# CDACHPCIE25/PPQSFLHE

Measured on AMD Instinct MI355X. Metric: ciphertexts/sec aggregated+PRE at N=2^16, L=12 RNS limbs, higher is better.
Workload: dtype u64

## Files before the change

include/mkckks.h:

```cpp
#ifndef MKCKKS_H
#define MKCKKS_H

#include <stddef.h>
#include <stdint.h>

#ifdef __cplusplus
extern "C" {
#endif

#define MKCKKS_OK 0
#define MKCKKS_E_INVALID (-1)
#define MKCKKS_E_NODEVICE (-2)
#define MKCKKS_E_HIP (-3)
#define MKCKKS_E_NOMEM (-4)
#define MKCKKS_E_INTERNAL (-5)
#define MKCKKS_E_PRECISION (-6)

typedef struct mkckks_ctx mkckks_ctx;

typedef struct mkckks_params {
    uint32_t log_n;
    uint32_t mult_depth;
    uint32_t scaling_bits;
    uint32_t first_bits;
// ... 32 lines not shown
int mkckks_host_free(mkckks_ctx *c, void *h_ptr);
int mkckks_upload_async(mkckks_ctx *c, void *d_dst, const void *h_src_pinned, size_t bytes, uint64_t *ticket_out);
int mkckks_download_async(mkckks_ctx *c, void *h_dst_pinned, const void *d_src, size_t bytes, uint64_t *ticket_out);
int mkckks_copy_done(mkckks_ctx *c, uint64_t ticket, int *done_out);
int mkckks_copy_wait(mkckks_ctx *c, uint64_t ticket);
int mkckks_fence_uploads(mkckks_ctx *c);
int mkckks_fence_compute(mkckks_ctx *c);
int mkckks_count_noncanonical(mkckks_ctx *c, const uint64_t *d_ct, uint32_t n_ct, uint32_t nl, uint64_t *h_count);

int mkckks_ntt_forward_batch(mkckks_ctx *c, uint64_t *d_polys, uint32_t n_polys, uint32_t nl, int with_p);
int mkckks_ntt_inverse_batch(mkckks_ctx *c, uint64_t *d_polys, uint32_t n_polys, uint32_t nl, int with_p);

int mkckks_eval_add_batch(mkckks_ctx *c, const uint64_t *d_a, const uint64_t *d_b, uint64_t *d_out,
                          uint32_t n_ct, uint32_t nl);
int mkckks_eval_sum_batch(mkckks_ctx *c, const uint64_t *d_in, uint64_t *d_out, uint32_t n_clients,
                          uint32_t n_ct, uint32_t nl);

int mkckks_rescale_mult_const_batch(mkckks_ctx *c, const uint64_t *d_in, uint64_t *d_out, uint32_t n_ct,
                                    uint32_t nl, double operand);
int mkckks_rescale_batch(mkckks_ctx *c, const uint64_t *d_in, uint64_t *d_out, uint32_t n_ct, uint32_t nl);
int mkckks_mult_const_batch(mkckks_ctx *c, uint64_t *d_ct, uint32_t n_ct, uint32_t nl, double operand);

int mkckks_mult_plain_batch(mkckks_ctx *c, uint64_t *d_ct, const uint64_t *d_pt, uint32_t n_ct, uint32_t n_pt, uint32_t nl);
int mkckks_mult_plain_rescale_batch(mkckks_ctx *c, const uint64_t *d_in, const uint64_t *d_pt, uint64_t *d_out, uint32_t n_ct,
                                    uint32_t n_pt, uint32_t nl);

int mkckks_reencrypt_batch(mkckks_ctx *c, const uint64_t *d_ct, const uint64_t *d_evk, uint64_t *d_out,
                           uint32_t n_ct, uint32_t nl);
int mkckks_reencrypt_accumulate_batch(mkckks_ctx *c, const uint64_t *d_ct, const uint64_t *d_evk, uint64_t *d_acc,
                                      uint32_t n_ct, uint32_t nl);
int mkckks_reencrypt_sum_batch(mkckks_ctx *c, const uint64_t *d_cts, const uint64_t *d_evks, uint64_t *d_out,
                               uint32_t n_clients, uint32_t n_ct, uint32_t nl);
int mkckks_q0_walk_choice(uint32_t row_tiles, uint32_t n_int_q, uint32_t n_idx, int mode);
int mkckks_scale_evk_batch(mkckks_ctx *c, const uint64_t *d_evk_in, uint64_t *d_evk_out, uint32_t n_keys,
                           const double *h_weights, uint32_t sf_level);
int mkckks_reencrypt_wsum_batch(mkckks_ctx *c, const uint64_t *d_cts, const uint64_t *d_evks_scaled, uint64_t *d_out,
                                uint32_t n_clients, uint32_t n_ct, uint32_t nl, const double *h_weights, uint32_t sf_level);
int mkckks_eval_wsum_batch(mkckks_ctx *c, const uint64_t *d_in, uint64_t *d_out, uint32_t n_terms, uint32_t n_ct, uint32_t nl,
                           const double *h_weights, uint32_t sf_level, int first_is_sum);
int mkckks_reencrypt_fanout_batch(mkckks_ctx *c, const uint64_t *d_ct, const uint64_t *d_evks, uint64_t *d_out,
                                  uint32_t n_keys, uint32_t n_ct, uint32_t nl);
int mkckks_compress_batch(mkckks_ctx *c, const uint64_t *d_in, uint64_t *d_out, uint32_t n_ct, uint32_t nl_in,
                          uint32_t nl_out);
int mkckks_reencrypt_fanout_compact_batch(mkckks_ctx *c, const uint64_t *d_ct, const uint64_t *d_evks, uint64_t *d_out,
                                          uint32_t n_keys, uint32_t n_ct, uint32_t nl_in, uint32_t nl_out);
int mkckks_modup_batch(mkckks_ctx *c, const uint64_t *d_c1, uint64_t *d_digits, uint32_t n, uint32_t nl);
int mkckks_moddown_batch(mkckks_ctx *c, const uint64_t *d_in, uint64_t *d_out, uint32_t n, uint32_t nl);

#define MKCKKS_SAMPLER_KEY_BYTES 32
int mkckks_sample_ternary(mkckks_ctx *c, int8_t *d_out, size_t count, const uint8_t *h_key32, uint32_t stream_id);
int mkckks_sample_gauss(mkckks_ctx *c, int32_t *d_out, size_t count, double sigma, const uint8_t *h_key32,
                        uint32_t stream_id);
int mkckks_sample_uniform(mkckks_ctx *c, uint64_t *d_out, uint32_t n_polys, uint32_t nl, int with_p,
                          const uint8_t *h_key32, uint32_t stream_id);
int mkckks_sample_gauss_wide(mkckks_ctx *c, int64_t *d_out, size_t count, double sigma, const uint8_t *h_key32,
                             uint32_t stream_id);
int mkckks_chacha20_block(mkckks_ctx *c, uint32_t *d_out16, const uint8_t *h_key32, uint32_t counter,
                          const uint32_t *h_nonce3);

int mkckks_keygen(mkckks_ctx *c, const int8_t *d_s, const uint64_t *d_a, const int32_t *d_e,
                  uint64_t *d_pk, uint64_t *d_sk);
int mkckks_rekeygen(mkckks_ctx *c, const int8_t *d_s_old, const uint64_t *d_pk_new, const int8_t *d_u,
                    const int32_t *d_e0, const int32_t *d_e1, uint64_t *d_evk);

int mkckks_encrypt_batch(mkckks_ctx *c, const uint64_t *d_pk, const uint64_t *d_pt, const int8_t *d_v,
                         const int32_t *d_e0, const int32_t *d_e1, uint64_t *d_ct, uint32_t n_ct, uint32_t nl);
// ... 100 lines not shown
```

ppqsflhe_amd/binding.py:

```python
import ctypes as C
import os

import numpy as np

_HERE = os.path.dirname(os.path.abspath(__file__))
_LIB = os.environ.get("MKCKKS_LIB") or os.path.join(_HERE, "libmkckks_hip.so")


class MkckksError(RuntimeError):
    def __init__(self, code, msg):
        super().__init__(f"mkckks error {code}: {msg}")
        self.code = code


class _Params(C.Structure):
    _fields_ = [("log_n", C.c_uint32), ("mult_depth", C.c_uint32), ("scaling_bits", C.c_uint32),
                ("first_bits", C.c_uint32), ("dnum", C.c_uint32), ("aux_bits", C.c_uint32),
                ("extra_bits", C.c_uint32), ("device", C.c_int32)]


class _Info(C.Structure):
    _fields_ = [("ring_dim", C.c_uint32), ("num_q", C.c_uint32), ("num_p", C.c_uint32),
                ("alpha", C.c_uint32), ("beta", C.c_uint32), ("slots", C.c_uint32)]

# ... 25 lines not shown
    "mkckks_fence_compute": (_int, [_vp]),
    "mkckks_count_noncanonical": (_int, [_vp, _vp, _u32, _u32, C.POINTER(C.c_uint64)]),
    "mkckks_debug_stamps": (_int, [_vp, _vp, _u32, C.POINTER(_sz)]),
    "mkckks_ntt_forward_batch": (_int, [_vp, _vp, _u32, _u32, _int]),
    "mkckks_ntt_inverse_batch": (_int, [_vp, _vp, _u32, _u32, _int]),
    "mkckks_eval_add_batch": (_int, [_vp, _vp, _vp, _vp, _u32, _u32]),
    "mkckks_eval_sum_batch": (_int, [_vp, _vp, _vp, _u32, _u32, _u32]),
    "mkckks_rescale_mult_const_batch": (_int, [_vp, _vp, _vp, _u32, _u32, _dbl]),
    "mkckks_rescale_batch": (_int, [_vp, _vp, _vp, _u32, _u32]),
    "mkckks_mult_const_batch": (_int, [_vp, _vp, _u32, _u32, _dbl]),
    "mkckks_mult_plain_batch": (_int, [_vp, _vp, _vp, _u32, _u32, _u32]),
    "mkckks_mult_plain_rescale_batch": (_int, [_vp, _vp, _vp, _vp, _u32, _u32, _u32]),
    "mkckks_reencrypt_batch": (_int, [_vp, _vp, _vp, _vp, _u32, _u32]),
    "mkckks_reencrypt_accumulate_batch": (_int, [_vp, _vp, _vp, _vp, _u32, _u32]),
    "mkckks_reencrypt_sum_batch": (_int, [_vp, _vp, _vp, _vp, _u32, _u32, _u32]),
    "mkckks_reencrypt_fanout_batch": (_int, [_vp, _vp, _vp, _vp, _u32, _u32, _u32]),
    "mkckks_scale_evk_batch": (_int, [_vp, _vp, _vp, _u32, _vp, _u32]),
    "mkckks_reencrypt_wsum_batch": (_int, [_vp, _vp, _vp, _vp, _u32, _u32, _u32, _vp, _u32]),
    "mkckks_eval_wsum_batch": (_int, [_vp, _vp, _vp, _u32, _u32, _u32, _vp, _u32, _int]),
    "mkckks_compress_batch": (_int, [_vp, _vp, _vp, _u32, _u32, _u32]),
    "mkckks_reencrypt_fanout_compact_batch": (_int, [_vp, _vp, _vp, _vp, _u32, _u32, _u32, _u32]),
    "mkckks_modup_batch": (_int, [_vp, _vp, _vp, _u32, _u32]),
    "mkckks_moddown_batch": (_int, [_vp, _vp, _vp, _u32, _u32]),
    "mkckks_keygen": (_int, [_vp, _vp, _vp, _vp, _vp, _vp]),
    "mkckks_rekeygen": (_int, [_vp, _vp, _vp, _vp, _vp, _vp, _vp]),
    "mkckks_keygen_join": (_int, [_vp, _vp, _vp, _vp, _vp, _vp]),
    "mkckks_partial_decrypt_batch": (_int, [_vp, _vp, _vp, _vp, _vp, _u32, _u32, _u32, _int]),
    "mkckks_fuse_shares_batch": (_int, [_vp, _vp, _vp, _u32, _u32, _u32]),
    "mkckks_switch_share_batch": (_int, [_vp, _vp, _vp, _vp, _vp, _vp, _vp, _vp, _u32, _u32, _u32, _int]),
    "mkckks_share_key": (_int, [_vp, _vp, _vp, _u32, _u32, _u32, C.c_char_p, _u32]),
    "mkckks_combine_key_shares": (_int, [_vp, _vp, _vp, _vp, _u32, _u32]),
    "mkckks_lagrange_at_zero": (_int, [_vp, _vp, _u32, _vp]),
    "mkckks_q0_walk_choice": (_int, [_u32, _u32, _u32, _int]),
    "mkckks_encrypt_batch": (_int, [_vp, _vp, _vp, _vp, _vp, _vp, _vp, _u32, _u32]),
    "mkckks_lift_ntt_batch": (_int, [_vp, _vp, _vp, _u32, _u32]),
    "mkckks_decrypt_batch": (_int, [_vp, _vp, _vp, _vp, _u32, _u32]),
    "mkckks_sample_ternary": (_int, [_vp, _vp, _sz, C.c_char_p, _u32]),
    "mkckks_sample_gauss": (_int, [_vp, _vp, _sz, _dbl, C.c_char_p, _u32]),
    "mkckks_sample_gauss_wide": (_int, [_vp, _vp, _sz, _dbl, C.c_char_p, _u32]),
    "mkckks_rerandomize_batch": (_int, [_vp, _vp, _vp, _vp, _vp, _vp, _vp, _u32, _u32, _u32]),
    "mkckks_sample_uniform": (_int, [_vp, _vp, _u32, _u32, _int, C.c_char_p, _u32]),
    "mkckks_chacha20_block": (_int, [_vp, _vp, C.c_char_p, _u32, C.POINTER(_u32)]),
    "mkckks_encrypt_seeded_batch": (_int, [_vp, _vp, _vp, _vp, _vp, _u32, _u32, C.c_char_p, _u32]),
    "mkckks_expand_seeded_batch": (_int, [_vp, _vp, _u32, _u32, C.c_char_p, C.POINTER(_u32)]),
    "mkckks_encode_batch": (_int, [_vp, _vp, _vp, _u32, _u32, _dbl]),
    "mkckks_decode_batch": (_int, [_vp, _vp, _vp, _u32, _u32, _dbl]),
    "mkckks_decode_flood_batch": (_int, [_vp, _vp, _vp, _u32, _u32, _dbl, C.c_char_p, _u32, _vp]),
    "mkckks_reduce_mod_batch": (_int, [_vp, _vp, _u32, _u32, _u32]),
    "mkckks_comm_unique_id": (_int, [_vp]),
    "mkckks_comm_create": (_int, [_vp, _vp, _int, _int, C.POINTER(_vp)]),
    "mkckks_comm_destroy": (_int, [_vp, _vp]),
    "mkckks_reduce_scatter_sum_mod": (_int, [_vp, _vp, _vp, _vp, _u32, _u32, _u32]),
    "mkckks_comm_library": (C.c_char_p, []),
    "mkckks_ctx_twiddles": (_int, [_vp, _u32, _int, _u64p]),
    "mkckks_debug_arith": (_int, [_vp, _u32, C.c_uint64, _vp, _vp, _sz]),
}
ARITH_OPS = {
    "csub": (0, 2, 1, 0),
    "add_mod": (1, 2, 1, 0),
    "sub_mod": (2, 2, 1, 0),
    "shoup_lazy": (3, 2, 1, 1),
    "shoup_mul": (4, 2, 1, 1),
    "mul_mod": (5, 2, 1, 0),
    "barrett_reduce128": (6, 2, 1, 0),
    "reduce_wide": (7, 2, 1, 0),
    "reduce_word": (8, 1, 1, 0),
# ... 474 lines not shown
```

ppqsflhe_amd/csrc/capi.cpp:

```cpp
#include <cstring>
#include <new>
#include <string>

#include "../../include/mkckks.h"
#include "comm.hpp"
#include "engine.hpp"

struct mkckks_ctx {
    mk::Engine *eng;
};

namespace {
thread_local std::string g_err;

template <typename F>
int guarded(F &&f) {
    try {
        f();
        return MKCKKS_OK;
    } catch (const mk::PrecisionError &e) {
        g_err = e.what();
        return MKCKKS_E_PRECISION;
    } catch (const mk::NoDevice &e) {
        g_err = e.what();
// ... 275 lines not shown
                                    uint32_t n_pt, uint32_t nl) {
    return guarded([&] {
        need(c && in && pt && out, "null argument");
        need(nl >= 2 && nl <= c->eng->params().L, "nl out of range");
        need(n_pt == 1 || n_pt == n_ct, "n_pt must be 1 or n_ct");
        c->eng->mult_plain_rescale(in, pt, out, n_ct, n_pt, nl);
    });
}

int mkckks_reencrypt_batch(mkckks_ctx *c, const uint64_t *ct, const uint64_t *evk, uint64_t *out, uint32_t n_ct,
                           uint32_t nl) {
    return guarded([&] {
        need(c && ct && evk && out, "null argument");
        c->eng->reencrypt(ct, evk, out, n_ct, nl);
    });
}
int mkckks_reencrypt_accumulate_batch(mkckks_ctx *c, const uint64_t *ct, const uint64_t *evk, uint64_t *acc,
                                      uint32_t n_ct, uint32_t nl) {
    return guarded([&] {
        need(c && ct && evk && acc, "null argument");
        c->eng->reencrypt(ct, evk, acc, n_ct, nl, true);
    });
}
int mkckks_reencrypt_sum_batch(mkckks_ctx *c, const uint64_t *cts, const uint64_t *evks, uint64_t *out, uint32_t n_clients,
                               uint32_t n_ct, uint32_t nl) {
    return guarded([&] {
        need(c && cts && evks && out, "null argument");
        c->eng->reencrypt_sum(cts, evks, out, n_clients, n_ct, nl);
    });
}
int mkckks_q0_walk_choice(uint32_t row_tiles, uint32_t n_int_q, uint32_t n_idx, int mode) {
    return mk::q0_walk_fused(row_tiles, n_int_q, n_idx, mode) ? 1 : 0;
}
int mkckks_scale_evk_batch(mkckks_ctx *c, const uint64_t *d_evk_in, uint64_t *d_evk_out, uint32_t n_keys,
                           const double *h_weights, uint32_t sf_level) {
    return guarded([&] {
        need(c && (n_keys == 0 || (d_evk_in && d_evk_out && h_weights)), "null argument");
        c->eng->scale_evk(d_evk_in, d_evk_out, n_keys, h_weights, sf_level);
    });
}
int mkckks_reencrypt_wsum_batch(mkckks_ctx *c, const uint64_t *d_cts, const uint64_t *d_evks_scaled, uint64_t *d_out,
                                uint32_t n_clients, uint32_t n_ct, uint32_t nl, const double *h_weights, uint32_t sf_level) {
    return guarded([&] {
        need(c && ((n_clients == 0 || n_ct == 0) || (d_cts && d_evks_scaled && d_out && h_weights)), "null argument");
        c->eng->reencrypt_wsum(d_cts, d_evks_scaled, d_out, n_clients, n_ct, nl, h_weights, sf_level);
    });
}
int mkckks_eval_wsum_batch(mkckks_ctx *c, const uint64_t *d_in, uint64_t *d_out, uint32_t n_terms, uint32_t n_ct, uint32_t nl,
                           const double *h_weights, uint32_t sf_level, int first_is_sum) {
    return guarded([&] {
        need(c && ((n_terms == 0 || n_ct == 0) || (d_in && d_out && h_weights)), "null argument");
        c->eng->eval_wsum(d_in, d_out, n_terms, n_ct, nl, h_weights, sf_level, first_is_sum != 0);
    });
}
int mkckks_reencrypt_fanout_batch(mkckks_ctx *c, const uint64_t *ct, const uint64_t *evks, uint64_t *out, uint32_t n_keys,
                                  uint32_t n_ct, uint32_t nl) {
    return guarded([&] {
        need(c && ct && evks && out, "null argument");
        need(nl >= 1 && nl <= c->eng->params().L, "nl out of range");
        if (!n_keys || !n_ct) return;
        c->eng->reencrypt_fanout(ct, evks, out, n_keys, n_ct, nl);
    });
}
static void need_compact_args(const mk::ParamSet &ps, const uint64_t *in, const uint64_t *out, uint32_t n_keys, uint32_t n_ct,
                              uint32_t nl_in, uint32_t nl_out) {
    need(nl_out >= 1 && nl_out < nl_in && nl_in <= ps.L, "need 1 <= nl_out < nl_in <= L");
// ... 292 lines not shown
```

ppqsflhe_amd/csrc/engine.hip:

```cpp
#include "engine.hpp"
#include "comm.hpp"
#include "dispatch.hpp"
#include "ntt_radix.hpp"
#include "qsum_kernels.hpp"
#include "fanout_kernels.hpp"
#include "codec_kernels.hpp"
#include "sampler_kernels.hpp"
#include "arith_probe_kernels.hpp"
#include "../../include/mkckks.h"

#include <cmath>
#include <cstdio>
#include <type_traits>
#include <cstdlib>
#include <cstring>

namespace mk {


template <bool INV>
__global__ __launch_bounds__(NTT_THREADS) void k_ntt_col(NttIo io, NttTables T, const u64 *scale,
                                                         const u64 *scale_sh) {
    extern __shared__ __attribute__((aligned(16))) u64 lds[];
    const uint32_t poly = blockIdx.y / io.nslots, s = blockIdx.y % io.nslots;
    if (ntt_slot_skipped(io, poly, io.vslot0 + s)) return;
    const uint32_t id = limb_id_of(io.vslot0 + s, io.nl, T.L);
    const LimbConst lc = T.limb[id];
    const uint32_t n = 1u << T.log_n, r1 = 1u << T.log_r1, r2 = 1u << T.log_r2;
    const u64 *src = io.in + (size_t)poly * io.in_stride + (size_t)(io.in_slot0 + s) * n;
    u64 *dst = io.out + (size_t)poly * io.out_stride + (size_t)(io.out_slot0 + s) * n;
    const uint32_t c0 = blockIdx.x * NTT_COLS;
    const uint32_t pairs = r1 * (NTT_COLS / 2);
    for (uint32_t e = threadIdx.x; e < pairs; e += NTT_THREADS) {
        const uint32_t r = e / (NTT_COLS / 2), cp = (e % (NTT_COLS / 2)) * 2;
        const ulong2 v = *reinterpret_cast<const ulong2 *>(src + (size_t)r * r2 + c0 + cp);
        lds[r * NTT_COLS + cp] = v.x;
        lds[r * NTT_COLS + cp + 1] = v.y;
    }
    __syncthreads();
    const u64 *tw = (INV ? T.itw : T.tw) + (size_t)id * n;
    const u64 *tw_sh = (INV ? T.itw_sh : T.tw_sh) + (size_t)id * n;
    lds_stages<INV>(lds, NTT_COLS, (int)T.log_r1, 1, NTT_COLS, true, tw, tw_sh, lc.q, lc.q2,
                    [](int) { return 1; });
// ... 466 lines not shown
    return msg + "): the one initialised second sees no device -- load the library that owns the device first (import torch "
                 "before libmkckks_hip.so, or link both against the same libamdhip64)";
}

static bool env_flag(const char *name, bool dflt) {
    const char *e = std::getenv(name);
    return e ? std::atoi(e) != 0 : dflt;
}
Knobs Knobs::from_env() {
    Knobs k;
    if (const char *e = std::getenv("MKCKKS_CHUNK")) {
        const int v = std::atoi(e);
        if (v >= 1 && v <= 64) k.chunk = (uint32_t)v;
    }
    if (const char *e = std::getenv("MKCKKS_QSUM_GROUP")) {
        const int v = std::atoi(e);
        if (v >= 1 && v <= 64) k.qsum_group = (uint32_t)v;
    }
    if (const char *e = std::getenv("MKCKKS_FANOUT_GROUP")) {
        const int v = std::atoi(e);
        if (v >= 1 && v <= 64) k.fanout_group = (uint32_t)v;
    }
    k.cu_affine = env_flag("MKCKKS_CU_AFFINE", k.cu_affine);
    k.generic_ntt = env_flag("MKCKKS_GENERIC_NTT", k.generic_ntt);
    k.no_pm = env_flag("MKCKKS_NO_PM", k.no_pm);
    k.no_fp64 = env_flag("MKCKKS_NO_FP64", k.no_fp64);
    if (const char *e = std::getenv("MKCKKS_Q0_WALK")) {
        if (!std::strcmp(e, "0")) k.q0_walk = 0;
        else if (!std::strcmp(e, "1")) k.q0_walk = 1;
    }
    if (const char *e = std::getenv("MKCKKS_PLAIN_FUSED")) {
        if (!std::strcmp(e, "0")) k.plain_fused = 0;
        else if (!std::strcmp(e, "1")) k.plain_fused = 1;
    }
    return k;
}

Engine::Engine(const ParamSet &ps, int device) : ps_(ps), device_(device), knobs_(Knobs::from_env()) {
    if (device_ < 0) return;
    int count = 0;
    if (hipGetDeviceCount(&count) != hipSuccess || count <= device_)
        throw NoDevice("no HIP device " + std::to_string(device_) + " (found " + std::to_string(count) + ")" +
                       hip_runtime_diagnosis());
    MK_HIP(hipSetDevice(device_));
    const uint32_t D = ps_.D, n = ps_.n;
    tabs_.log_n = ps_.log_n;
    tabs_.log_r1 = (ps_.log_n % 2 == 0) ? ((ps_.log_n / 2) & ~1u) : ps_.log_n / 2;
    tabs_.log_r2 = ps_.log_n - tabs_.log_r1;
    if (knobs_.generic_ntt) { tabs_.log_r1 = ps_.log_n / 2; tabs_.log_r2 = ps_.log_n - tabs_.log_r1; }
    const bool radix_both = fast_log_h(tabs_.log_r1, 1u << tabs_.log_r2) && fast_row(tabs_.log_r2, 1u << tabs_.log_r1);
    const bool fp_ok = radix_both && !knobs_.no_fp64;
    tabs_.has_fp = 0;
    fp_of_.assign(D, 0);
    for (uint32_t i = 0; i < D; ++i) {
        ps_.limb[i].fp = (fp_ok && ps_.moduli[i] < (5ull << 48)) ? 1u : 0u;
        fp_of_[i] = (uint8_t)ps_.limb[i].fp;
        tabs_.has_fp |= ps_.limb[i].fp;
    }
    bool all_pm = radix_both && !knobs_.no_pm;
    for (uint32_t i = 0; i < D; ++i)
        if (!ps_.limb[i].fp && !pm_eligible(ps_.moduli[i])) all_pm = false;
    tabs_.int_pm = all_pm ? 1u : 0u;
    for (uint32_t i = 0; i < D; ++i) {
        const bool pm = all_pm && !ps_.limb[i].fp;
        ps_.limb[i].pm = pm ? 1u : 0u;
        ps_.limb[i].pm_c = pm ? (uint32_t)(((u64)1 << ps_.limb[i].k) - ps_.moduli[i]) : 0u;
// ... 338 lines not shown
    ClassMasks m;
    if (classes & 1) m.integer = class_mask(io, T.h_fp_of, T.L, false);
    if (classes & 2) m.fp = class_mask(io, T.h_fp_of, T.L, true);
    return m;
}
static ClassMasks limb_classes(uint32_t nl, const NttTables &T) {
    NttIo sel{};
    sel.nslots = sel.nl = nl;
    return slot_classes(sel, T);
}
static ClassMasks target_classes(const DevConv &cv, const NttTables &T, unsigned classes = 3) {
    ClassMasks m;
    for (uint32_t j = 0; j < cv.n_out; ++j) {
        const bool fp = T.h_fp_of[cv.dst_id[j]] != 0;
        if (fp && (classes & 2)) m.fp |= 1ull << j;
        if (!fp && (classes & 1)) m.integer |= 1ull << j;
    }
    return m;
}

template <typename F>
static void for_each_class(const NttTables &T, const ClassMasks &m, F &&f) {
    if (m.integer) with_int_arith(T, [&](auto ar) { f(ar, m.integer, (uint32_t)__builtin_popcountll(m.integer)); });
    if (m.fp) f(std::integral_constant<int, AR_FP>{}, m.fp, (uint32_t)__builtin_popcountll(m.fp));
}

template <int LOG_H>
static uint32_t col_tiles(const NttTables &T) { return (1u << T.log_r2) / (256u >> LOG_H); }
template <int LOG_H>
static uint32_t row_tiles(const NttTables &T) { return (1u << T.log_r1) / (256u >> LOG_H); }

template <bool INV>
static void launch_col(const NttIo &io0, const NttTables &T, uint32_t n_polys, const u64 *scale, const u64 *scale_sh,
                       hipStream_t s, int pack = 0) {
    const uint32_t r1 = 1u << T.log_r1, r2 = 1u << T.log_r2;
    const bool radix = dispatch<2, 3, 4>(fast_log_h(T.log_r1, r2), [&](auto log_h) {
        constexpr int LOG_H = decltype(log_h)::value;
        for_each_class(T, slot_classes(io0, T), [&](auto ar, unsigned long long mask, uint32_t nsel) {
            NttIo io = io0;
            io.slot_mask = mask;
            io.nsel = nsel;
            k_ntt_col_r<LOG_H, INV, decltype(ar)::value>
                <<<dim3(col_tiles<LOG_H>(T), n_polys * nsel), NTT_THREADS, 0, s>>>(io, T, scale, scale_sh, pack);
        });
    });
    if (radix) return;
    if (pack) throw std::logic_error("packed output needs the radix column kernel");
    k_ntt_col<INV><<<dim3(r2 / NTT_COLS, n_polys * io0.nslots), NTT_THREADS, (size_t)r1 * NTT_COLS * sizeof(u64), s>>>(
        io0, T, scale, scale_sh);
}

static bool row_tail_supported(const NttTables &T) { return fast_row(T.log_r2, 1u << T.log_r1) != 0; }

template <bool INV>
static void launch_row(const NttIo &io0, const NttTables &T, uint32_t n_polys, const TailArgs &tail, hipStream_t s,
                       unsigned classes = 3) {
    const uint32_t n = 1u << T.log_n, r1 = 1u << T.log_r1;
    const bool radix = dispatch<2, 3, 4, 9>(fast_row(T.log_r2, r1), [&](auto row_h) {
        constexpr int ROW_H = decltype(row_h)::value;
        for_each_class(T, slot_classes(io0, T, classes), [&](auto ar, unsigned long long mask, uint32_t nsel) {
            NttIo io = io0;
            io.slot_mask = mask;
            io.nsel = nsel;
            if constexpr (ROW_H == 9)
                k_ntt_row3<INV, decltype(ar)::value><<<dim3((r1 / 4) * n_polys * nsel), NTT_THREADS, 0, s>>>(io, T, tail);
            else
                k_ntt_row_r<ROW_H, INV, decltype(ar)::value>
                    <<<dim3(row_tiles<ROW_H>(T) * n_polys * nsel), NTT_THREADS, 0, s>>>(io, T, tail);
        });
    });
    if (radix) return;
    if (tail.enabled) throw std::logic_error("fused tail needs the radix row kernel");
    const uint32_t tile = n < (uint32_t)NTT_TILE ? n : (uint32_t)NTT_TILE;
    k_ntt_row<INV><<<dim3(n / tile, n_polys * io0.nslots), NTT_THREADS, (size_t)tile * sizeof(u64), s>>>(io0, T);
}

static void ntt_passes(NttIo io, const NttTables &T, uint32_t n_polys, bool inverse, const u64 *scale,
                       const u64 *scale_sh, hipStream_t s, int pack = 0) {
    if (n_polys == 0 || io.nslots == 0) return;
    NttIo second = io;
    second.in_group = 0;
    second.in = io.out;
    second.in_stride = io.out_stride;
    second.in_slot0 = io.out_slot0;
    const TailArgs none{};
    if (!inverse) {
        launch_col<false>(io, T, n_polys, nullptr, nullptr, s);
        launch_row<false>(second, T, n_polys, none, s);
    } else {
        launch_row<true>(io, T, n_polys, none, s);
        launch_col<true>(second, T, n_polys, scale, scale_sh, s, pack);
    }
    MK_HIP(hipGetLastError());
}

template <int LOG_H, int N_IN, int SRCMODE>
static void launch_conv_col_n(const ConvIo &io0, const NttTables &T, const DevConv &cv, hipStream_t s, unsigned classes) {
    for_each_class(T, target_classes(cv, T, classes), [&](auto ar, unsigned long long mask, uint32_t nsel) {
        ConvIo io = io0;
        io.target_mask = mask;
        io.nsel = nsel;
        if constexpr (LOG_H >= 3)
            k_conv_col2<LOG_H, N_IN, decltype(ar)::value, DevConv, SRCMODE>
                <<<dim3(io.items * col_tiles<LOG_H>(T) * ((nsel + 1) / 2)), NTT_THREADS, 0, s>>>(io, T, cv);
        else
            k_conv_col<LOG_H, N_IN, decltype(ar)::value, DevConv, SRCMODE>
                <<<dim3(io.items * col_tiles<LOG_H>(T) * nsel), NTT_THREADS, 0, s>>>(io, T, cv);
    });
}
template <int LOG_H, int N_IN>
static void launch_conv_col_m(const ConvIo &io, const NttTables &T, const DevConv &cv, hipStream_t s, int srcmode,
                              unsigned classes) {
    if constexpr (N_IN <= 4 && LOG_H >= 3) {
        if (srcmode == 1) return launch_conv_col_n<LOG_H, N_IN, 1>(io, T, cv, s, classes);
        if (srcmode == 2) return launch_conv_col_n<LOG_H, N_IN, (N_IN > 1 ? 2 : 0)>(io, T, cv, s, classes);
    }
    if (srcmode != 0) throw std::logic_error("double conversion sources: unsupported shape");
    launch_conv_col_n<LOG_H, N_IN, 0>(io, T, cv, s, classes);
}
static bool launch_conv_col(const ConvIo &io, const NttTables &T, const DevConv &cv, hipStream_t s, int srcmode = 0,
                            unsigned classes = 3) {
    const bool radix = dispatch<2, 3, 4>(fast_log_h(T.log_r1, 1u << T.log_r2), [&](auto log_h) {
        if (!dispatch<1, 2, 3, 4, 5, 6, 7, 8>(cv.n_in, [&](auto n_in) {
                launch_conv_col_m<decltype(log_h)::value, decltype(n_in)::value>(io, T, cv, s, srcmode, classes);
            }))
            throw std::invalid_argument("base conversion fan-in unsupported");
    });
    if (radix) MK_HIP(hipGetLastError());
    return radix;
}
template <int LOG_H, int N_IN>
static void launch_conv_col_psum_n(const ConvIo &io0, const NttTables &T, const DevConv &cv, hipStream_t s) {
    for_each_class(T, target_classes(cv, T), [&](auto ar, unsigned long long mask, uint32_t nsel) {
        ConvIo io = io0;
        io.target_mask = mask;
        io.nsel = nsel;
        if constexpr (decltype(ar)::value == AR_FP)
            k_conv_col_psum2<LOG_H, N_IN, DevConv>
                <<<dim3(io.items * col_tiles<LOG_H>(T) * ((nsel + 1) / 2)), NTT_THREADS, 0, s>>>(io, T, cv);
        else
            k_conv_col_psum<LOG_H, N_IN, decltype(ar)::value, DevConv>
                <<<dim3(io.items * col_tiles<LOG_H>(T) * nsel), NTT_THREADS, 0, s>>>(io, T, cv);
    });
}
static void launch_conv_col_psum(const ConvIo &io, const NttTables &T, const DevConv &cv, hipStream_t s) {
    if (!dispatch<3, 4>(fast_log_h(T.log_r1, 1u << T.log_r2), [&](auto log_h) {
            if (!dispatch<1, 2, 3, 4, 5, 6, 7, 8>(cv.n_in, [&](auto n_in) {
                    launch_conv_col_psum_n<decltype(log_h)::value, decltype(n_in)::value>(io, T, cv, s);
                }))
                throw std::invalid_argument("base conversion fan-in unsupported");
        }))
        throw std::logic_error("summed conversion needs 64- or 256-point columns");
    MK_HIP(hipGetLastError());
}
static void launch_icol_sum(const u64 *pc, u64 *psum, const NttTables &T, uint32_t K, uint32_t n_polys, uint32_t n_clients,
                            size_t in_cstride, hipStream_t s) {
    if (!dispatch<3, 4>(fast_log_h(T.log_r1, 1u << T.log_r2), [&](auto log_h) {
            constexpr int LOG_H = decltype(log_h)::value;
            with_int_arith(T, [&](auto ar) {
                k_icol_sum<LOG_H, decltype(ar)::value><<<dim3(col_tiles<LOG_H>(T), n_polys * K), NTT_THREADS, 0, s>>>(
                    pc, psum, T, K, n_clients, in_cstride);
            });
// ... 273 lines not shown
        for (size_t i = 0; i < t.src.size(); ++i) put(t.src[i], t.hatinv[i]);
    }
    BaseConvTable t = ps_.moddown_table(nl);
    for (size_t i = 0; i < t.src.size(); ++i) put(t.src[i], t.hatinv[i]);
    return limb_vector(key, v);
}

const u64 *Engine::p_inverse(uint32_t nl) {
    const std::string key = "pinv_" + std::to_string(nl);
    auto it = vec_cache_.find(key);
    if (it != vec_cache_.end()) return it->second;
    std::vector<u64> pinv(2 * nl);
    for (uint32_t i = 0; i < nl; ++i) {
        pinv[i] = ps_.p_inv_mod(i);
        pinv[nl + i] = h_shoup(pinv[i], ps_.moduli[i]);
    }
    return limb_vector(key, pinv);
}

void Engine::modup_core(const u64 *c1, size_t c1_stride, u64 *coef, u64 *dig, uint32_t cnt, uint32_t nl,
                        bool rows_int_only, uint32_t in_group, size_t in_gstride, bool p_scaled) {
    const uint32_t n = ps_.n, ext = nl + ps_.K, nparts = ps_.num_parts(nl), D = ps_.D;
    const u64 *fold = folded_scale(nl);
    bool fused = fast_log_h(tabs_.log_r1, 1u << tabs_.log_r2) != 0;
    NttIo s1{c1, coef, c1_stride, (size_t)nl * n, 0, 0, 0, nl, nl};
    s1.in_group = in_group;
    s1.in_gstride = in_gstride;
    const size_t dstride = (size_t)nparts * ext * n;
    bool doubles = fused && tabs_.has_fp && fast_log_h(tabs_.log_r1, 1u << tabs_.log_r2) >= 3;
    for (uint32_t part = 0; part < nparts && doubles; ++part) {
        const DevConv &cv = modup_conv(nl, part, p_scaled);
        if (conv_src_mode(cv) < 0 || (conv_src_mode(cv) != 0 && cv.n_in > 4)) doubles = false;
    }
    ntt_passes(s1, tabs_, cnt, true, fold, fold + D, stream_, fused ? (doubles ? 2 : 1) : 0);
    for (uint32_t part = 0; part < nparts && fused; ++part) {
        ConvIo io{coef, dig + (size_t)part * ext * n, (size_t)nl * n, dstride, cnt, 0, 0};
        const DevConv &cv = modup_conv(nl, part, p_scaled);
        launch_conv_col(io, tabs_, cv, stream_, doubles ? conv_src_mode(cv) : 0);
    }
    if (fused) {
        NttIo row{dig, dig, (size_t)ext * n, (size_t)ext * n, 0, 0, 0, ext, nl, nparts, ps_.alpha};
        if (!skip_rows_) launch_row<false>(row, tabs_, cnt * nparts, TailArgs{}, stream_, rows_int_only ? 1u : 3u);
        MK_HIP(hipGetLastError());
        return;
    }
    if (rows_int_only || p_scaled) throw std::logic_error("fused inner product needs the radix kernels");
    for (uint32_t part = 0; part < nparts; ++part) {
        const DevConv &cv = modup_conv(nl, part);
        const uint32_t lo = part * ps_.alpha, hi = lo + cv.n_in;
        u64 *d = dig + (size_t)part * ext * n;
        launch_baseconv(coef, (size_t)nl * n, d, dstride, cv, d_limb_, n, cnt, 1, stream_);
        if (lo > 0) {
            NttIo a{d, d, dstride, dstride, 0, 0, 0, lo, nl};
            ntt_passes(a, tabs_, cnt, false, nullptr, nullptr, stream_);
        }
        if (hi < ext) {
            NttIo b{d, d, dstride, dstride, hi, hi, hi, ext - hi, nl};
            ntt_passes(b, tabs_, cnt, false, nullptr, nullptr, stream_);
        }
    }
}

void Engine::moddown_convert(const u64 *til, u64 *pc, u64 *conv, uint32_t cnt, uint32_t nl, bool rows_done) {
    const uint32_t n = ps_.n, K = ps_.K, ext = nl + K, D = ps_.D;
    const u64 *fold = folded_scale(nl);
    NttIo s5{til, pc, (size_t)ext * n, (size_t)K * n, nl, 0, nl, K, nl};
    const DevConv &cv = moddown_conv(nl);
    if (!rows_done) {
        ntt_passes(s5, tabs_, cnt, true, fold, fold + D, stream_, 1);
    } else {
        NttIo second = s5;
// ... 1212 lines not shown
```

ppqsflhe_amd/csrc/engine.hpp:

```cpp
#pragma once
#include <hip/hip_runtime.h>

#include <map>
#include <stdexcept>
#include <string>
#include <utility>
#include <vector>

#include "modarith.hpp"
#include "ntt_kernels.hpp"
#include "params.hpp"

namespace mk {

constexpr uint32_t SHAMIR_MAX_PARTIES = 64;

struct HipError : std::runtime_error {
    using std::runtime_error::runtime_error;
};
struct NoDevice : std::runtime_error {
    using std::runtime_error::runtime_error;
};
struct PrecisionError : std::runtime_error {
    using std::runtime_error::runtime_error;
// ... 3 lines not shown
    do {                                                                                          \
        hipError_t _e = (expr);                                                                   \
        if (_e != hipSuccess)                                                                     \
            throw mk::HipError(std::string(#expr) + ": " + hipGetErrorString(_e) + " (" __FILE__ \
                               ":" + std::to_string(__LINE__) + ")");                             \
    } while (0)

constexpr int MAX_CONV_IN = 8;
constexpr int MAX_CONV_OUT = 40;

struct DevConv {
    uint32_t n_in, n_out;
    uint32_t src_id[MAX_CONV_IN];
    uint32_t src_slot[MAX_CONV_IN];
    uint32_t dst_id[MAX_CONV_OUT];
    uint32_t dst_slot[MAX_CONV_OUT];
    u64 hatinv[MAX_CONV_IN], hatinv_sh[MAX_CONV_IN];
    const u64 *hat;
    const double *hat_d;
    const double *hatq_d;
    const double *hat30_d;
};

struct Knobs {
    uint32_t chunk = 16;
    uint32_t fanout_group = 7;
    uint32_t qsum_group = 8;
    bool cu_affine = true;
    bool generic_ntt = false;
    bool no_pm = false;
    bool no_fp64 = false;
    int q0_walk = 2;
    int plain_fused = 2;
    static Knobs from_env();
};

constexpr uint32_t Q0_WALK_MIN_GRID = 512;
inline bool q0_walk_fused(uint32_t tiles, uint32_t nsel, uint32_t cnt, int mode) {
    if (mode == 0 || mode == 1) return mode == 1;
    return (uint64_t)tiles * nsel * cnt >= Q0_WALK_MIN_GRID;
}

class Engine {
public:
    explicit Engine(const ParamSet &ps, int device);
    ~Engine();
    Engine(const Engine &) = delete;
    Engine &operator=(const Engine &) = delete;

    const ParamSet &params() const { return ps_; }
    bool has_device() const { return device_ >= 0; }
    int device() const { return device_; }
    void set_stream(hipStream_t s) { stream_ = s; }
    hipStream_t stream() const { return stream_; }
    void sync();

    void *dev_alloc(size_t bytes);
    void dev_free(void *p);
    void upload(void *d, const void *h, size_t bytes);
    void download(void *h, const void *d, size_t bytes);
    void *host_alloc(size_t bytes);
    void host_free(void *p);
    uint64_t upload_async(void *d, const void *h, size_t bytes);
    uint64_t download_async(void *h, const void *d, size_t bytes);
    bool copy_done(uint64_t ticket);
    void copy_wait(uint64_t ticket);
    void fence_uploads();
    void fence_compute();
    uint64_t count_noncanonical(const u64 *ct, uint32_t n_ct, uint32_t nl);

    void ntt_forward(u64 *d, uint32_t n_polys, uint32_t nl, bool with_p);
    void ntt_inverse(u64 *d, uint32_t n_polys, uint32_t nl, bool with_p);

// ... 128 lines not shown
```

ppqsflhe_amd/csrc/ntt_radix.hpp:

```cpp
#pragma once
#include "modarith.hpp"
#include "ntt_kernels.hpp"

namespace mk {

#ifndef MK_NT8
#define MK_NT8 0
#endif
MK_D u64 ld_stream(const u64 *p) { return (MK_NT && MK_NT8) ? __builtin_nontemporal_load(p) : *p; }
MK_D ulong2 ld_stream2(const ulong2 *p) {
    if (MK_NT) {
        ulong2 v;
        v.x = __builtin_nontemporal_load(&p->x);
        v.y = __builtin_nontemporal_load(&p->y);
        return v;
    }
    return *p;
}
MK_D u64 ld_pass(const u64 *p) { return (MK_NT >= 2 && MK_NT8) ? __builtin_nontemporal_load(p) : *p; }
#ifndef MK_NT8S
#define MK_NT8S 1
#endif
MK_D void st_pass(u64 *p, u64 v) {
    if (MK_NT >= 2 && MK_NT8S) __builtin_nontemporal_store(v, p);
// ... 751 lines not shown
    u64 ring[DEPTH][N_IN];
#pragma unroll
    for (int k = 0; k < DEPTH; ++k)
#pragma unroll
        for (int i = 0; i < N_IN; ++i) ring[k][i] = src[(size_t)cv.src_slot[i] * n + (size_t)(j + H * k) * r2];
#pragma unroll
    for (int k = 0; k < H; ++k) {
        u64 p[N_IN];
#pragma unroll
        for (int i = 0; i < N_IN; ++i) p[i] = ring[k % DEPTH][i];
        if (k + DEPTH < H) {
#pragma unroll
            for (int i = 0; i < N_IN; ++i)
                ring[k % DEPTH][i] = src[(size_t)cv.src_slot[i] * n + (size_t)(j + H * (k + DEPTH)) * r2];
        }
        uint32_t a0[N_IN], a1[N_IN];
        if (!((AR == AR_FP) && SRCMODE != 0)) conv_split_sources<N_IN, SRCMODE>(p, a0, a1);
        double s_lo = 0.0, s_hi = 0.0;
        conv_halves_d<AR, SRCMODE>(p[0], s_lo, s_hi);
        xa[k] = conv_output<N_IN, AR, SRCMODE>(p, a0, a1, ka, la, s_lo, s_hi);
        xb[k] = conv_output<N_IN, AR, SRCMODE>(p, a0, a1, kb, lb, s_lo, s_hi);
        asm volatile("" : "+v"(xa[k]), "+v"(xb[k]));
        __builtin_amdgcn_sched_barrier(0);
    }
    }
    u64 *dst = io.out + (size_t)item * io.out_stride + (size_t)cv.dst_slot[jta] * n + tile * S + c;
    col_forward_finish<LOG_H, AR>(xa, lds, T.tw + (size_t)ida * n, T.tw_sh + (size_t)ida * n, la, j, c, dst, r2);
    if (!two) return;
    __syncthreads();
    dst = io.out + (size_t)item * io.out_stride + (size_t)cv.dst_slot[jtb] * n + tile * S + c;
    const u64 *twb = T.tw + (size_t)idb * n, *twb_sh = T.tw_sh + (size_t)idb * n;
    asm volatile("" : "+s"(twb), "+s"(twb_sh));
    col_forward_finish<LOG_H, AR>(xb, lds, twb, twb_sh, lb, j, c, dst, r2);
}

template <int LOG_H, int AR>
__global__ __launch_bounds__(NTT_THREADS, 3) void k_icol_sum(const u64 *pc, u64 *psum, NttTables T, uint32_t K,
                                                             uint32_t n_clients, size_t in_cstride) {
    using TL = ColTile<LOG_H>;
    constexpr int H = TL::H, S = TL::S;
    static_assert(AR != AR_FP, "P limbs are integer-class");
    __shared__ u64 lds[TL::WORDS + ColTwB<LOG_H>::WORDS];
    const uint32_t poly = blockIdx.y / K, k = blockIdx.y % K;
    const uint32_t id = T.L + k;
    const LimbConst lc = T.limb[id];
    const uint32_t n = 1u << T.log_n, r2 = 1u << T.log_r2;
    const int c = threadIdx.x % S, j = threadIdx.x / S;
    const size_t off = ((size_t)poly * K + k) * n + blockIdx.x * S + c;
    const u64 *itw0 = T.itw + (size_t)id * n, *itw_sh0 = T.itw_sh + (size_t)id * n;
    u64 acc[H];
#pragma unroll
    for (int kk = 0; kk < H; ++kk) acc[kk] = 0;
    ColTwB<LOG_H>::stage(lds + TL::WORDS, itw0, itw_sh0);
    wave_lds_sync();
    const u64 *strip = lds + TL::WORDS;
#pragma unroll 1
    for (uint32_t cl = 0; cl < n_clients; ++cl) {
        const u64 *src = pc + (size_t)cl * in_cstride + off;
        u64 x[H];
        uint32_t r2v = r2;
        asm volatile("" : "+s"(r2v));
#pragma unroll
        for (int kk = 0; kk < H; ++kk) x[kk] = ld_pass(src + (uint32_t)(H * j + kk) * r2v);
        radix_inverse_staged<LOG_H, AR>(x, [&](int i) { return ColTwB<LOG_H>::pair_b(strip, j, i); }, lc);
        if (cl) __syncthreads();
#pragma unroll
// ... 1746 lines not shown
```

Baseline: 32830.

## Fuse inverse column NTT of FP limbs with modup base conversion into one kernel

Adds k_icol_conv, which runs the inverse column NTT for the fp-class source limbs, writes the scaled coefficients back, and accumulates base-conversion partial sums for a few fp targets. It then runs the forward column NTT for those targets in the same kernel. The separate inverse column pass and conversion-column launch skip those slots and targets through masks. The aim is to avoid re-reading coefficients from global memory and to cut launches. The cost is a heavier kernel with more registers and an extra accumulation path, and by default it only turns on for large grids with one target.

```diff
diff --git a/include/mkckks.h b/include/mkckks.h
--- a/include/mkckks.h
+++ b/include/mkckks.h
@@ -88,6 +88,7 @@
 int mkckks_reencrypt_sum_batch(mkckks_ctx *c, const uint64_t *d_cts, const uint64_t *d_evks, uint64_t *d_out,
                                uint32_t n_clients, uint32_t n_ct, uint32_t nl);
 int mkckks_q0_walk_choice(uint32_t row_tiles, uint32_t n_int_q, uint32_t n_idx, int mode);
+uint32_t mkckks_icol_conv_targets(uint32_t n_fp_targets, uint64_t grid, int mode);
 int mkckks_scale_evk_batch(mkckks_ctx *c, const uint64_t *d_evk_in, uint64_t *d_evk_out, uint32_t n_keys,
                            const double *h_weights, uint32_t sf_level);
 int mkckks_reencrypt_wsum_batch(mkckks_ctx *c, const uint64_t *d_cts, const uint64_t *d_evks_scaled, uint64_t *d_out,
diff --git a/ppqsflhe_amd/binding.py b/ppqsflhe_amd/binding.py
--- a/ppqsflhe_amd/binding.py
+++ b/ppqsflhe_amd/binding.py
@@ -81,6 +81,7 @@
     "mkckks_combine_key_shares": (_int, [_vp, _vp, _vp, _vp, _u32, _u32]),
     "mkckks_lagrange_at_zero": (_int, [_vp, _vp, _u32, _vp]),
     "mkckks_q0_walk_choice": (_int, [_u32, _u32, _u32, _int]),
+    "mkckks_icol_conv_targets": (_u32, [_u32, C.c_uint64, _int]),
     "mkckks_encrypt_batch": (_int, [_vp, _vp, _vp, _vp, _vp, _vp, _vp, _u32, _u32]),
     "mkckks_lift_ntt_batch": (_int, [_vp, _vp, _vp, _u32, _u32]),
     "mkckks_decrypt_batch": (_int, [_vp, _vp, _vp, _vp, _u32, _u32]),
diff --git a/ppqsflhe_amd/csrc/capi.cpp b/ppqsflhe_amd/csrc/capi.cpp
--- a/ppqsflhe_amd/csrc/capi.cpp
+++ b/ppqsflhe_amd/csrc/capi.cpp
@@ -331,6 +331,9 @@
 int mkckks_q0_walk_choice(uint32_t row_tiles, uint32_t n_int_q, uint32_t n_idx, int mode) {
     return mk::q0_walk_fused(row_tiles, n_int_q, n_idx, mode) ? 1 : 0;
 }
+uint32_t mkckks_icol_conv_targets(uint32_t n_fp_targets, uint64_t grid, int mode) {
+    return mk::icol_conv_targets(n_fp_targets, grid, mode);
+}
 int mkckks_scale_evk_batch(mkckks_ctx *c, const uint64_t *d_evk_in, uint64_t *d_evk_out, uint32_t n_keys,
                            const double *h_weights, uint32_t sf_level) {
     return guarded([&] {
diff --git a/ppqsflhe_amd/csrc/engine.hip b/ppqsflhe_amd/csrc/engine.hip
--- a/ppqsflhe_amd/csrc/engine.hip
+++ b/ppqsflhe_amd/csrc/engine.hip
@@ -9,6 +9,7 @@
 #include "arith_probe_kernels.hpp"
 #include "../../include/mkckks.h"
 
+#include <algorithm>
 #include <cmath>
 #include <cstdio>
 #include <type_traits>
@@ -541,6 +542,9 @@
     if (const char *e = std::getenv("MKCKKS_PLAIN_FUSED")) {
         if (!std::strcmp(e, "0")) k.plain_fused = 0;
         else if (!std::strcmp(e, "1")) k.plain_fused = 1;
+    }
+    if (const char *e = std::getenv("MKCKKS_ICOL_CONV")) {
+        if (e[0] >= '0' && e[0] <= '3' && !e[1]) k.icol_conv = e[0] - '0';
     }
     return k;
 }
@@ -945,11 +949,14 @@
 
 template <bool INV>
 static void launch_col(const NttIo &io0, const NttTables &T, uint32_t n_polys, const u64 *scale, const u64 *scale_sh,
-                       hipStream_t s, int pack = 0) {
+                       hipStream_t s, int pack = 0, unsigned long long skip = 0) {
     const uint32_t r1 = 1u << T.log_r1, r2 = 1u << T.log_r2;
     const bool radix = dispatch<2, 3, 4>(fast_log_h(T.log_r1, r2), [&](auto log_h) {
         constexpr int LOG_H = decltype(log_h)::value;
-        for_each_class(T, slot_classes(io0, T), [&](auto ar, unsigned long long mask, uint32_t nsel) {
+        ClassMasks m = slot_classes(io0, T);
+        m.integer &= ~skip;
+        m.fp &= ~skip;
+        for_each_class(T, m, [&](auto ar, unsigned long long mask, uint32_t nsel) {
             NttIo io = io0;
             io.slot_mask = mask;
             io.nsel = nsel;
@@ -958,7 +965,7 @@
         });
     });
     if (radix) return;
-    if (pack) throw std::logic_error("packed output needs the radix column kernel");
+    if (pack || skip) throw std::logic_error("packed output needs the radix column kernel");
     k_ntt_col<INV><<<dim3(r2 / NTT_COLS, n_polys * io0.nslots), NTT_THREADS, (size_t)r1 * NTT_COLS * sizeof(u64), s>>>(
         io0, T, scale, scale_sh);
 }
@@ -989,7 +996,7 @@
 }
 
 static void ntt_passes(NttIo io, const NttTables &T, uint32_t n_polys, bool inverse, const u64 *scale,
-                       const u64 *scale_sh, hipStream_t s, int pack = 0) {
+                       const u64 *scale_sh, hipStream_t s, int pack = 0, unsigned long long icol_skip = 0) {
     if (n_polys == 0 || io.nslots == 0) return;
     NttIo second = io;
     second.in_group = 0;
@@ -1002,14 +1009,18 @@
         launch_row<false>(second, T, n_polys, none, s);
     } else {
         launch_row<true>(io, T, n_polys, none, s);
-        launch_col<true>(second, T, n_polys, scale, scale_sh, s, pack);
+        launch_col<true>(second, T, n_polys, scale, scale_sh, s, pack, icol_skip);
     }
     MK_HIP(hipGetLastError());
 }
 
 template <int LOG_H, int N_IN, int SRCMODE>
-static void launch_conv_col_n(const ConvIo &io0, const NttTables &T, const DevConv &cv, hipStream_t s, unsigned classes) {
-    for_each_class(T, target_classes(cv, T, classes), [&](auto ar, unsigned long long mask, uint32_t nsel) {
+static void launch_conv_col_n(const ConvIo &io0, const NttTables &T, const DevConv &cv, hipStream_t s, unsigned classes,
+                              unsigned long long done) {
+    ClassMasks m = target_classes(cv, T, classes);
+    m.integer &= ~done;
+    m.fp &= ~done;
+    for_each_class(T, m, [&](auto ar, unsigned long long mask, uint32_t nsel) {
         ConvIo io = io0;
         io.target_mask = mask;
         io.nsel = nsel;
@@ -1023,24 +1034,37 @@
 }
 template <int LOG_H, int N_IN>
 static void launch_conv_col_m(const ConvIo &io, const NttTables &T, const DevConv &cv, hipStream_t s, int srcmode,
-                              unsigned classes) {
+                              unsigned classes, unsigned long long done) {
     if constexpr (N_IN <= 4 && LOG_H >= 3) {
-        if (srcmode == 1) return launch_conv_col_n<LOG_H, N_IN, 1>(io, T, cv, s, classes);
-        if (srcmode == 2) return launch_conv_col_n<LOG_H, N_IN, (N_IN > 1 ? 2 : 0)>(io, T, cv, s, classes);
+        if (srcmode == 1) return launch_conv_col_n<LOG_H, N_IN, 1>(io, T, cv, s, classes, done);
+        if (srcmode == 2) return launch_conv_col_n<LOG_H, N_IN, (N_IN > 1 ? 2 : 0)>(io, T, cv, s, classes, done);
     }
     if (srcmode != 0) throw std::logic_error("double conversion sources: unsupported shape");
-    launch_conv_col_n<LOG_H, N_IN, 0>(io, T, cv, s, classes);
+    launch_conv_col_n<LOG_H, N_IN, 0>(io, T, cv, s, classes, done);
 }
 static bool launch_conv_col(const ConvIo &io, const NttTables &T, const DevConv &cv, hipStream_t s, int srcmode = 0,
-                            unsigned classes = 3) {
+                            unsigned classes = 3, unsigned long long done = 0) {
     const bool radix = dispatch<2, 3, 4>(fast_log_h(T.log_r1, 1u << T.log_r2), [&](auto log_h) {
         if (!dispatch<1, 2, 3, 4, 5, 6, 7, 8>(cv.n_in, [&](auto n_in) {
-                launch_conv_col_m<decltype(log_h)::value, decltype(n_in)::value>(io, T, cv, s, srcmode, classes);
+                launch_conv_col_m<decltype(log_h)::value, decltype(n_in)::value>(io, T, cv, s, srcmode, classes, done);
             }))
             throw std::invalid_argument("base conversion fan-in unsupported");
     });
     if (radix) MK_HIP(hipGetLastError());
     return radix;
+}
+static void launch_icol_conv(const IcolConvIo &io, const NttTables &T, uint32_t nt_max, const u64 *scale, const u64 *scale_sh,
+                             hipStream_t s) {
+    if (!dispatch<3, 4>(fast_log_h(T.log_r1, 1u << T.log_r2), [&](auto log_h) {
+            constexpr int LOG_H = decltype(log_h)::value;
+            if (!dispatch<1, 2, 3>(nt_max, [&](auto nt_c) {
+                    k_icol_conv<LOG_H, decltype(nt_c)::value>
+                        <<<dim3(io.njobs * io.items * col_tiles<LOG_H>(T)), NTT_THREADS, 0, s>>>(io, T, scale, scale_sh);
+                }))
+                throw std::logic_error("k_icol_conv takes 1 to 3 targets");
+        }))
+        throw std::logic_error("k_icol_conv needs 64- or 256-point columns");
+    MK_HIP(hipGetLastError());
 }
 template <int LOG_H, int N_IN>
 static void launch_conv_col_psum_n(const ConvIo &io0, const NttTables &T, const DevConv &cv, hipStream_t s) {
@@ -1380,11 +1404,67 @@
         const DevConv &cv = modup_conv(nl, part, p_scaled);
         if (conv_src_mode(cv) < 0 || (conv_src_mode(cv) != 0 && cv.n_in > 4)) doubles = false;
     }
-    ntt_passes(s1, tabs_, cnt, true, fold, fold + D, stream_, fused ? (doubles ? 2 : 1) : 0);
+    std::vector<unsigned long long> icol_done(nparts, 0);
+    IcolConvIo icol{coef, dig, (size_t)nl * n, dstride, cnt, 0, {}};
+    uint32_t icol_nt_max = 0;
+    unsigned long long icol_slots = 0;
+    if (doubles && knobs_.icol_conv != 0 && nparts <= (uint32_t)ICOL_MAX_JOBS) {
+        std::vector<unsigned long long> fp_targets(nparts, 0);
+        uint32_t eligible = 0;
+        for (uint32_t part = 0; part < nparts; ++part) {
+            const DevConv &cv = modup_conv(nl, part, p_scaled);
+            if (conv_src_mode(cv) != 1) continue;
+            fp_targets[part] = target_classes(cv, tabs_, 2).fp;
+            eligible += fp_targets[part] != 0;
+        }
+        const uint64_t grid = (uint64_t)cnt * eligible * ((1u << tabs_.log_r2) / (256u >> (tabs_.log_r1 / 2)));
+        std::vector<IcolJob> jobs;
+        for (uint32_t part = 0; part < nparts; ++part) {
+            const DevConv &cv = modup_conv(nl, part, p_scaled);
+            IcolJob jb{};
+            uint32_t first_fp = 0;
+            for (uint32_t i = 0; i < cv.n_in; ++i)
+                if (fp_of_[cv.src_id[i]]) {
+                    if (!jb.n_in) first_fp = i;
+                    jb.src_id[jb.n_in] = cv.src_id[i];
+                    jb.src_slot[jb.n_in++] = cv.src_slot[i];
+                    icol_slots |= 1ull << cv.src_slot[i];
+                }
+            if (!jb.n_in) continue;
+            unsigned long long m = fp_targets[part];
+            uint32_t nt = icol_conv_targets((uint32_t)__builtin_popcountll(m), grid, knobs_.icol_conv);
+            for (; nt; --nt, m &= m - 1) icol_done[part] |= m & (~m + 1);
+            for (unsigned long long d = icol_done[part]; d; d &= d - 1) {
+                const uint32_t t = (uint32_t)__builtin_ctzll(d);
+                jb.dst_id[jb.nt] = cv.dst_id[t];
+                jb.dst_slot[jb.nt] = cv.dst_slot[t];
+                jb.hat_d[jb.nt] = cv.hat_d + t;
+                jb.hatq_d[jb.nt++] = cv.hatq_d + t;
+            }
+            for (uint32_t t = jb.nt; t < 3; ++t) {
+                jb.dst_id[t] = jb.src_id[0];
+                jb.hat_d[t] = cv.hat_d + (size_t)first_fp * cv.n_out;
+                jb.hatq_d[t] = cv.hatq_d + (size_t)first_fp * cv.n_out;
+            }
+            jb.hat_stride = cv.n_out;
+            jb.dig_off = (size_t)part * ext * n;
+            icol_nt_max = std::max(icol_nt_max, jb.nt);
+            jobs.push_back(jb);
+        }
+        if (icol_nt_max) {
+            std::stable_sort(jobs.begin(), jobs.end(),
+                             [](const IcolJob &a, const IcolJob &b) { return a.n_in + a.nt > b.n_in + b.nt; });
+            for (const IcolJob &jb : jobs) icol.job[icol.njobs++] = jb;
+        } else {
+            icol_slots = 0;
+        }
+    }
+    ntt_passes(s1, tabs_, cnt, true, fold, fold + D, stream_, fused ? (doubles ? 2 : 1) : 0, icol_slots);
+    if (icol_slots) launch_icol_conv(icol, tabs_, icol_nt_max, fold, fold + D, stream_);
     for (uint32_t part = 0; part < nparts && fused; ++part) {
         ConvIo io{coef, dig + (size_t)part * ext * n, (size_t)nl * n, dstride, cnt, 0, 0};
         const DevConv &cv = modup_conv(nl, part, p_scaled);
-        launch_conv_col(io, tabs_, cv, stream_, doubles ? conv_src_mode(cv) : 0);
+        launch_conv_col(io, tabs_, cv, stream_, doubles ? conv_src_mode(cv) : 0, 3, icol_done[part]);
     }
     if (fused) {
         NttIo row{dig, dig, (size_t)ext * n, (size_t)ext * n, 0, 0, 0, ext, nl, nparts, ps_.alpha};
diff --git a/ppqsflhe_amd/csrc/engine.hpp b/ppqsflhe_amd/csrc/engine.hpp
--- a/ppqsflhe_amd/csrc/engine.hpp
+++ b/ppqsflhe_amd/csrc/engine.hpp
@@ -59,6 +59,7 @@
     bool no_fp64 = false;
     int q0_walk = 2;
     int plain_fused = 2;
+    int icol_conv = -1;
     static Knobs from_env();
 };
 
@@ -66,6 +67,15 @@
 inline bool q0_walk_fused(uint32_t tiles, uint32_t nsel, uint32_t cnt, int mode) {
     if (mode == 0 || mode == 1) return mode == 1;
     return (uint64_t)tiles * nsel * cnt >= Q0_WALK_MIN_GRID;
+}
+
+constexpr uint32_t ICOL_CONV_MAX = 3, ICOL_CONV_AUTO_MAX = 1, ICOL_CONV_MIN_GRID = 2048;
+inline uint32_t icol_conv_targets(uint32_t n_fp, uint64_t grid, int mode) {
+    if (mode >= 0 && mode <= (int)ICOL_CONV_MAX) return (uint32_t)mode < n_fp ? (uint32_t)mode : n_fp;
+    if (grid < ICOL_CONV_MIN_GRID) return 0;
+    for (uint32_t nt = ICOL_CONV_AUTO_MAX < n_fp ? ICOL_CONV_AUTO_MAX : n_fp; nt >= 1; --nt)
+        if ((n_fp - nt) % 2 == 0) return nt;
+    return 0;
 }
 
 class Engine {
diff --git a/ppqsflhe_amd/csrc/ntt_radix.hpp b/ppqsflhe_amd/csrc/ntt_radix.hpp
--- a/ppqsflhe_amd/csrc/ntt_radix.hpp
+++ b/ppqsflhe_amd/csrc/ntt_radix.hpp
@@ -807,6 +807,112 @@
     const u64 *twb = T.tw + (size_t)idb * n, *twb_sh = T.tw_sh + (size_t)idb * n;
     asm volatile("" : "+s"(twb), "+s"(twb_sh));
     col_forward_finish<LOG_H, AR>(xb, lds, twb, twb_sh, lb, j, c, dst, r2);
+}
+
+MK_D double uniform_d(double v) {
+    const u64 b = dbits(v);
+    const uint32_t lo = __builtin_amdgcn_readfirstlane((uint32_t)b), hi = __builtin_amdgcn_readfirstlane((uint32_t)(b >> 32));
+    return bitsd(((u64)hi << 32) | lo);
+}
+struct IcolJob {
+    uint32_t n_in, nt;
+    uint32_t src_id[4], src_slot[4];
+    uint32_t dst_id[3], dst_slot[3];
+    const double *hat_d[3], *hatq_d[3];
+    uint32_t hat_stride;
+    size_t dig_off;
+};
+constexpr int ICOL_MAX_JOBS = 6;
+struct IcolConvIo {
+    u64 *coef;
+    u64 *dig;
+    size_t coef_stride, dig_stride;
+    uint32_t items, njobs;
+    IcolJob job[ICOL_MAX_JOBS];
+};
+#ifndef MK_ICOL_CONV_WAVES3
+#define MK_ICOL_CONV_WAVES3 2
+#endif
+template <int LOG_H, int NT>
+__global__ __launch_bounds__(NTT_THREADS, NT == 3 ? MK_ICOL_CONV_WAVES3 : (NT == 2 ? 3 : 4)) void k_icol_conv(IcolConvIo io, NttTables T,
+                                                                                                          const u64 *scale,
+                                                                                                          const u64 *scale_sh) {
+    using TL = ColTile<LOG_H>;
+    constexpr int H = TL::H, S = TL::S;
+    static_assert(NT >= 1 && NT <= 3, "1..3 targets");
+    __shared__ u64 lds[TL::WORDS + ColTwB<LOG_H>::WORDS];
+    const uint32_t n = 1u << T.log_n, r2 = 1u << T.log_r2, tiles = r2 / S;
+    const uint32_t groups = io.items * tiles;
+    const uint32_t jidx = blockIdx.x / groups;
+    const IcolJob &jb = io.job[jidx];
+    uint32_t grp, mem, item, tile;
+    group_member(blockIdx.x % groups, groups, 1, T.cu_affine, grp, mem);
+    conv_item_tile(grp, groups, io.items, tiles, item, tile);
+    const u64 *strip = lds + TL::WORDS;
+    const uint32_t nt = jb.nt, n_in = jb.n_in;
+    double qt[NT], acc[NT][H];
+#pragma unroll
+    for (int t = 0; t < NT; ++t) {
+        qt[t] = T.limb[jb.dst_id[t]].qd;
+#pragma unroll
+        for (int k = 0; k < H; ++k) acc[t][k] = 0.0;
+    }
+#pragma unroll 1
+    for (uint32_t i = 0; i < n_in; ++i) {
+        const uint32_t id = jb.src_id[i];
+        const LimbConst lc = T.limb[id];
+        uint32_t r2v = r2, tid = threadIdx.x;
+        asm volatile("" : "+s"(r2v));
+        asm volatile("" : "+v"(tid));
+        const int c = tid % S, j = tid / S;
+        u64 *p = io.coef + (size_t)item * io.coef_stride + (size_t)jb.src_slot[i] * n + tile * S + c;
+        if (i) __syncthreads();
+        ColTwB<LOG_H>::stage(lds + TL::WORDS, T.itw + (size_t)id * n, T.itw_sh + (size_t)id * n);
+        u64 x[H];
+#pragma unroll
+        for (int k = 0; k < H; ++k) x[k] = ld_pass(p + (uint32_t)(H * j + k) * r2v);
+        wave_lds_sync();
+        radix_inverse_staged<LOG_H, AR_FP>(x, [&](int e) { return ColTwB<LOG_H>::pair_b(strip, j, e); }, lc);
+#pragma unroll
+        for (int k = 0; k < H; ++k) lds[TL::at(j, k, c)] = x[k];
+        __syncthreads();
+#pragma unroll
+        for (int k = 0; k < H; ++k) x[k] = lds[TL::at(k, j, c)];
+        radix_inverse_staged<LOG_H, AR_FP>(x, [&](int e) { return ColTwB<LOG_H>::pair_a(strip, e); }, lc);
+        const double sc = bitsd(scale[id]), sc_q = bitsd(scale_sh[id]);
+        double hd[NT], hq[NT];
+#pragma unroll
+        for (int t = 0; t < NT; ++t) {
+            hd[t] = uniform_d(jb.hat_d[t][i * jb.hat_stride]);
+            hq[t] = uniform_d(jb.hatq_d[t][i * jb.hat_stride]);
+        }
+#pragma unroll
+        for (int k = 0; k < H; ++k) {
+            double sd = fp_mulmod(bitsd(x[k]), sc, sc_q, lc.qd);
+            sd = sd < 0.0 ? sd + lc.qd : sd;
+            st_pass(p + (uint32_t)(j + H * k) * r2v, dbits(sd));
+#pragma unroll
+            for (int t = 0; t < NT; ++t) acc[t][k] += fp_mulmod(sd, hd[t], hq[t], qt[t]);
+#pragma unroll
+            for (int t = 0; t < NT; ++t) asm volatile("" : "+v"(acc[t][k]));
+            __builtin_amdgcn_sched_barrier(0);
+        }
+    }
+#pragma unroll
+    for (int t = 0; t < NT; ++t) {
+        if ((uint32_t)t >= nt) break;
+        const uint32_t idt = jb.dst_id[t];
+        const LimbConst lt = T.limb[idt];
+        const int c = threadIdx.x % S, j = threadIdx.x / S;
+        u64 x[H];
+#pragma unroll
+        for (int k = 0; k < H; ++k) x[k] = dbits(fp_reduce(acc[t][k], lt.qd, lt.qinv));
+        __syncthreads();
+        const u64 *tw = T.tw + (size_t)idt * n, *tw_sh = T.tw_sh + (size_t)idt * n;
+        asm volatile("" : "+s"(tw), "+s"(tw_sh));
+        u64 *dst = io.dig + (size_t)item * io.dig_stride + jb.dig_off + (size_t)jb.dst_slot[t] * n + tile * S + c;
+        col_forward_finish<LOG_H, AR_FP>(x, lds, tw, tw_sh, lt, j, c, dst, r2);
+    }
 }
 
 template <int LOG_H, int AR>
```

Result: faster. 33590, median of 6 (+2.3%).
